# BarryFutureman/EvolutionaryDistributedTraining

Measured on AMD Instinct MI355X. Metric: GB/s of param bytes reduced per outer step (device-resident), 1/2/4/8 GPUs, higher is better.
Workload: dtype f32

## Files before the change

evolutionarydistributedtraining_amd/_lib.py:

```python
from __future__ import annotations

import ctypes
import os

import torch

PKG_DIR = os.path.dirname(os.path.abspath(__file__))
LIB_PATH = os.path.join(PKG_DIR, "libedt_sync.so")

EDT_F32 = 0
EDT_BF16 = 1
EDT_MAX_WORKERS = 64
EDT_MXFP8 = 0
EDT_MXFP4 = 1
EDT_ROUND_NEAREST = 0
EDT_ROUND_STOCHASTIC = 1
EDT_ABI_VERSION = 6

_DT = {torch.float32: EDT_F32, torch.bfloat16: EDT_BF16}

_P = ctypes.c_void_p
_U64 = ctypes.c_uint64
_I = ctypes.c_int
_D = ctypes.c_double
SIGNATURES = [
    ("edt_outer_step", _I, [_P, _I, ctypes.POINTER(_P), _I, _I, _P, _I, _U64, _D, _D, _I, _P]),
    ("edt_outer_step_bcast", _I, [_P, _I, ctypes.POINTER(_P), _I, _I, _P, _I, _U64, _D, _D, _I,
                                  ctypes.POINTER(_P), _I, _P]),
    ("edt_outer_step_tail", _I, [_P, _I, ctypes.POINTER(_P), _I, _I, _P, _I, _U64, _D, _D, _I, _P, _P]),
    ("edt_outer_step_scaled", _I, [_P, _I, ctypes.POINTER(_P), _I, _I, _P, _I, _U64, _D, _D, _I, _P,
                                   ctypes.c_float, _P]),
    ("edt_delta_stats_doubles", _U64, [_I, ctypes.c_int64]),
    ("edt_delta_stats", _I, [_P, _I, ctypes.POINTER(_P), _I, _I, _U64, _P, ctypes.c_int64, _P, _P]),
    ("edt_pair_merge_tail", _I, [_P, _P, _P, _P, _I, _P, _I, _P, _P, _I, _U64, _D, _D, _I, _P, _P]),
    ("edt_outer_step_ws", _I, [_P, _I, ctypes.POINTER(_P), _I, _I, _P, _I, _U64, _D, _D, _I, _P, _P]),
    ("edt_outer_list_workspace_bytes", _U64, [_I, _I]),
    ("edt_outer_step_list", _I, [ctypes.POINTER(_P), _I, ctypes.POINTER(_P), _I, _I, ctypes.POINTER(_P), _I,
                                 ctypes.POINTER(_U64), _I, _D, _D, _I, _P, _U64, _P]),
    ("edt_outer_step_list_tail", _I, [ctypes.POINTER(_P), _I, ctypes.POINTER(_P), _I, _I, ctypes.POINTER(_P), _I,
                                      ctypes.POINTER(_U64), _I, _D, _D, _I, _P, ctypes.POINTER(_U64), _P, _U64, _P]),
    ("edt_outer_step_list_scaled", _I, [ctypes.POINTER(_P), _I, ctypes.POINTER(_P), _I, _I, ctypes.POINTER(_P), _I,
                                        ctypes.POINTER(_U64), _I, _D, _D, _I, _P, ctypes.POINTER(_U64),
                                        ctypes.c_float, _P, _U64, _P]),
    ("edt_delta_stats_list_workspace_bytes", _U64, [_I, _I]),
    ("edt_delta_stats_list", _I, [ctypes.POINTER(_P), _I, ctypes.POINTER(_P), _I, _I, ctypes.POINTER(_U64), _I, _P,
                                  ctypes.c_int64, _P, _P, _U64, _P]),
    ("edt_delta_partial", _I, [_P, _I, ctypes.POINTER(_P), _I, _I, _I, _U64, _P, _I, _P]),
    ("edt_sgd_apply", _I, [_P, _I, _P, _P, _I, _U64, _D, _D, _I, _P]),
    ("edt_sgd_apply_sum", _I, [_P, _I, ctypes.POINTER(_P), _I, _P, _I, _U64, _D, _D, _I, _P]),
    ("edt_sgd_apply_scaled", _I, [_P, _I, _P, _P, _I, _U64, _D, _D, _I, ctypes.c_float, _P]),
    ("edt_sgd_apply_sum_scaled", _I, [_P, _I, ctypes.POINTER(_P), _I, _P, _I, _U64, _D, _D, _I, ctypes.c_float, _P]),
    ("edt_partial_sum_stats_doubles", _U64, [ctypes.c_int64]),
    ("edt_partial_sum_stats", _I, [ctypes.POINTER(_P), _I, _I, _U64, _P, ctypes.c_int64, _P, _P]),
    ("edt_q_region_bytes", _U64, [_U64, _I]),
    ("edt_delta_partial_q", _I, [_P, _I, ctypes.POINTER(_P), _I, _I, _I, _U64, _U64, _I, _P, _P, _P]),
    ("edt_sgd_apply_sum_q", _I, [_P, _I, ctypes.POINTER(_P), _I, _I, _P, _I, _U64, _D, _D, _I, _P]),
# ... 171 lines not shown
```

evolutionarydistributedtraining_amd/csrc/edt_outer.hip:

```cpp
#include "edt_step.h"

namespace {


struct Workers {
    const void* p[EDT_MAX_WORKERS];
};

struct OuterArgs {
    void* theta;
    void* mom;
    float* acc_out;
    uint64_t n;
    int K;
    float kdiv;
    float kinv;
    int div_exact;
    int accumulate;
    void* acc_ws;
    int acc_in;
    int acc_store;
    SgdScalars sgd;
    Workers w;
    Workers bc;
// ... 183 lines not shown
};

template <int GDT, int N, bool SC = false, class... S>
__global__ __launch_bounds__(kBlock) void sgd_apply_sum_kernel(void* theta, Partials P, int np, void* mom,
                                                               uint64_t n, SgdScalars s, S... scale) {
    static_assert(sizeof...(S) == (SC ? 1 : 0), "one grad_scale with SC, none without");
    for_vec_tail<N>(n, [&](auto tagN, uint64_t i) {
        constexpr int M = decltype(tagN)::value;
        float g0[M], g[M];
        sgd_from_sum<GDT, M, SC>(theta, mom, i, s, np, [&](int r, float (&x)[M]) { ld<EDT_F32, M>(P.p[r], i, x); }, g0, g,
                                 scale...);
        st<GDT, M>(theta, i, g);
    });
}

template <int GDT, int N, bool SC = false, class... S>
__global__ __launch_bounds__(kBlock) void sgd_apply_kernel(void* theta, const float* acc, void* mom,
                                                           uint64_t n, SgdScalars s, S... scale) {
    static_assert(sizeof...(S) == (SC ? 1 : 0), "one grad_scale with SC, none without");
    for_vec_tail<N>(n, [&](auto tagN, uint64_t i) {
        constexpr int M = decltype(tagN)::value;
        float g0[M], g[M];
        sgd_from_sum<GDT, M, SC>(theta, mom, i, s, 1, [&](int, float (&x)[M]) { ld<EDT_F32, M>(acc, i, x); }, g0, g,
                                 scale...);
        st<GDT, M>(theta, i, g);
    });
}



template <int GDT, int WDT, int KC, int N, int H2 = 4>
__device__ __forceinline__ void probe_elems(const OuterArgs& a, uint64_t i) {
    float g[N], b[N], acc[N];
    ld<GDT, N, false, H2>(a.theta, i, g);
    ld<GDT, N, false, H2>(a.mom, i, b);
#pragma unroll
    for (int j = 0; j < N; ++j) acc[j] = 0.f;
    const int K = KC > 0 ? KC : a.K;
#pragma unroll 8
    for (int k = 0; k < K; ++k) {
        float w[N];
        ld<WDT, N, nt_worker_loads<WDT, H2>(), H2>(a.wp(k), i, w);
#pragma unroll
        for (int j = 0; j < N; ++j) acc[j] += w[j];
    }
#pragma unroll
// ... 455 lines not shown
    return sgd_apply_sum_impl<false>(theta_g, gdt, acc_f32, nacc, momentum, has_momentum, n, lr, momentum_coef, nesterov,
                                     1.f, stream);
}

int edt_sgd_apply_sum_scaled(void* theta_g, int gdt, const float* const* acc_f32, int nacc, void* momentum,
                             int has_momentum, uint64_t n, double lr, double momentum_coef, int nesterov,
                             float grad_scale, void* stream) {
    return sgd_apply_sum_impl<true>(theta_g, gdt, acc_f32, nacc, momentum, has_momentum, n, lr, momentum_coef, nesterov,
                                    grad_scale, stream);
}

int edt_sgd_apply(void* theta_g, int gdt, const float* acc_f32, void* momentum, int has_momentum,
                  uint64_t n, double lr, double momentum_coef, int nesterov, void* stream) {
    return sgd_apply_impl<false>(theta_g, gdt, acc_f32, momentum, has_momentum, n, lr, momentum_coef, nesterov, 1.f,
                                 stream);
}

int edt_sgd_apply_scaled(void* theta_g, int gdt, const float* acc_f32, void* momentum, int has_momentum,
                         uint64_t n, double lr, double momentum_coef, int nesterov, float grad_scale, void* stream) {
    return sgd_apply_impl<true>(theta_g, gdt, acc_f32, momentum, has_momentum, n, lr, momentum_coef, nesterov,
                                grad_scale, stream);
}

}
```

evolutionarydistributedtraining_amd/csrc/edt_stats.hip:

```cpp
#include "edt_chunksum.h"
#include "edt_mx.h"
#include "edt_step.h"

namespace {

constexpr int kStatsGroup = 8;
constexpr int kStatsUpc = kTileSlots / kWavesPerBlock;
constexpr int kStatsMaxWidth = 3 * EDT_MAX_WORKERS + 2;

__host__ __device__ constexpr int stats_width(int K) { return 3 * K + 2; }

struct StatsWorkers {
    const void* p[EDT_MAX_WORKERS];
};

struct StatsArgs {
    const void* theta;
    const uint64_t* chunks;
    double* rows;
    uint64_t units;
    uint64_t u0;
    int K;
    float kdiv;
    float kinv;
    StatsWorkers w;
    static constexpr bool kList = false;
    __device__ __forceinline__ const StatsArgs& operands(uint64_t) const { return *this; }
    __device__ __forceinline__ const void* th() const { return theta; }
    __device__ __forceinline__ const void* wp(int k) const { return w.p[k]; }
};

struct StatsListArgs;
struct TensorOperands {
    const StatsListArgs& a;
    uint64_t t;
    __device__ __forceinline__ const void* th() const;
    __device__ __forceinline__ const void* wp(int k) const;
};

struct StatsListArgs {
    const void* const* theta;
    const void* const* w;
    const uint64_t* vec;
    const uint64_t* chunks;
    double* rows;
    uint64_t units;
    uint64_t u0;
    uint64_t T;
    int K;
    float kdiv;
    float kinv;
    static constexpr bool kList = true;
    __device__ __forceinline__ TensorOperands operands(uint64_t c) const { return {*this, chunks[3 * c + 2]}; }
};
__device__ __forceinline__ const void* TensorOperands::th() const { return a.theta[t]; }
__device__ __forceinline__ const void* TensorOperands::wp(int k) const { return a.w[(uint64_t)k * a.T + t]; }


template <int DT, bool VEC, bool NT>
__device__ __forceinline__ void ld8(const void* p, uint64_t i, float (&x)[kVec]) {
    if constexpr (VEC) {
        ld<DT, kVec, NT>(p, i, x);
    } else {
#pragma unroll
        for (int j = 0; j < kVec; ++j) {
            float y[1];
            ld<DT, 1>(p, i + j, y);
            x[j] = y[0];
        }
    }
}

template <int N>
__device__ __forceinline__ void mask_count(float (&x)[N], double& count) {
#pragma unroll
    for (int j = 0; j < N; ++j) {
        const bool bad = (__float_as_uint(x[j]) & 0x7fffffffu) >= 0x7f800000u;
        if (bad) {
            x[j] = 0.f;
            count += 1.0;
        }
    }
}

template <int N>
__device__ __forceinline__ void dot_chain(const float (&x)[N], const float (&y)[N], double& s) {
#pragma unroll
    for (int j = 0; j < N; ++j) s = __builtin_fma((double)x[j], (double)y[j], s);
}

template <int GDT, int WDT, int DIV, int KC, bool KM, bool VEC, class Args>
__global__ __launch_bounds__(kBlock) void delta_stats_kernel(Args a) {
// ... 34 lines not shown
        for (int q = 0; q < G; ++q) {
#pragma unroll
            for (int j = 0; j < kVec; ++j) d[q][j] = 0.f;
            de[q][0] = 0.f;
            if (KC > 0 ? q < KC : k0 + q < K) {
                if (has_vec) ld8<WDT, VEC, NT>(o.wp(k0 + q), i, d[q]);
                if (has_edge) ld<WDT, 1>(o.wp(k0 + q), e, de[q]);
            }
        }
#pragma unroll
        for (int q = 0; q < G; ++q) {
            if (KC > 0 ? q < KC : k0 + q < K) {
                delta_of<GDT>(d[q], g);
                mean_add<GDT, DIV, true>(a, d[q], acc);
                delta_of<GDT>(de[q], ge);
                mean_add<GDT, DIV, true>(a, de[q], acce);
                mask_count(d[q], ck[q]);
                mask_count(de[q], ck[q]);
                dot_chain(d[q], d[q], skk[q]);
                dot_chain(de[q], de[q], skk[q]);
            }
        }
        if constexpr (KM) {
            mask_count(acc, cm);
            mask_count(acce, cm);
            dot_chain(acc, acc, smm);
            dot_chain(acce, acce, smm);
#pragma unroll
            for (int q = 0; q < G; ++q) {
                dot_chain(d[q], acc, skm[q]);
                dot_chain(de[q], acce, skm[q]);
            }
            double v[3 * G + 2], r[Red<3 * G + 2>::N2];
            v[0] = smm;
            v[2 * G + 1] = cm;
#pragma unroll
            for (int q = 0; q < G; ++q) {
                v[1 + q] = skk[q];
                v[1 + G + q] = skm[q];
                v[2 * G + 2 + q] = ck[q];
            }
            tile_reduce<3 * G + 2>(v, r);
            red_store<3 * G + 2>(r, [&](int idx, double x) {
                if (idx == 0) row[0] = x;
                else if (idx <= G) { if (idx - 1 < K) row[idx] = x; }
                else if (idx <= 2 * G) { if (idx - 1 - G < K) row[K + idx - G] = x; }
                else if (idx == 2 * G + 1) row[2 * K + 1] = x;
                else if (idx - 2 * G - 2 < K) row[2 * K + idx - 2 * G] = x;
            });
        } else {
            double v[2 * G], r[Red<2 * G>::N2];
#pragma unroll
            for (int q = 0; q < G; ++q) {
                v[q] = skk[q];
                v[G + q] = ck[q];
            }
            tile_reduce<2 * G>(v, r);
            red_store<2 * G>(r, [&](int idx, double x) {
                const int k = k0 + (idx < G ? idx : idx - G);
                if (k < K) row[(idx < G ? 1 : 2 * K + 2) + k] = x;
            });
        }
    }
    if constexpr (!KM) {
        mask_count(acc, cm);
        mask_count(acce, cm);
        dot_chain(acc, acc, smm);
        dot_chain(acce, acce, smm);
        const double v[2] = {smm, cm};
        double r[Red<2>::N2];
        tile_reduce<2>(v, r);
        red_store<2>(r, [&](int idx, double x) { row[idx == 0 ? 0 : 2 * K + 1] = x; });
    }
    __syncthreads();
    const int W = stats_width(K);
    double* out = a.rows + unit_slot(u, a.units) * (uint64_t)W;
    for (int q = threadIdx.x; q < W; q += kBlock) {
        double x = 0.0;
        if (KM || q <= K || q > 2 * K) x = (part[0][q] + part[1][q]) + (part[2][q] + part[3][q]);
        out[q] = x;
    }
}

template <int GDT, int WDT, int DIV, int KC, bool KM, bool VEC, class A>
int launch_stats(A a, hipStream_t s) {
    const uint64_t units = a.units;
    for (uint64_t u0 = 0; u0 < units; u0 += kUnitGridCap) {
// ... 142 lines not shown
    const double v[2] = {smm, cm};
    double r[Red<2>::N2];
    tile_reduce<2>(v, r);
    red_store<2>(r, [&](int idx, double x) { part[wave][idx] = x; });
    __syncthreads();
    double* out = a.rows + unit_slot(u, a.units) * (uint64_t)kPartialStatsWidth;
    if (threadIdx.x < kPartialStatsWidth) {
        const int q = threadIdx.x;
        out[q] = (part[0][q] + part[1][q]) + (part[2][q] + part[3][q]);
    }
}

template <int GDT, int FMT, int NPC>
int launch_partial_stats_q(PartialStatsQArgs a, hipStream_t s) {
    const uint64_t units = a.units;
    for (uint64_t u0 = 0; u0 < units; u0 += kUnitGridCap) {
        a.u0 = u0;
        partial_sum_stats_q_kernel<GDT, FMT, NPC><<<unit_grid(units - u0), kBlock, 0, s>>>(a);
        if (int rc = check_launch("partial_sum_stats_q_kernel")) return rc;
    }
    return EDT_OK;
}

}

extern "C" {

uint64_t edt_partial_sum_stats_doubles(int64_t nchunks) {
    if (nchunks < 0) return 0;
    return (uint64_t)nchunks * (uint64_t)kPartialStatsWidth * (1ull + kStatsUpc);
}

int edt_partial_sum_stats(const float* const* acc_f32, int nacc, int gdt, uint64_t n, const uint64_t* chunk_desc,
                          int64_t nchunks, double* out, void* stream) {
    g_err[0] = 0;
    int rc = check_master_dtype(gdt);
    if (!rc) rc = check_partial_count(nacc);
    if (rc) return rc;
    if (nchunks < 0) return fail(EDT_ERR_ARG, "negative chunk count");
    if (!acc_f32) return fail(EDT_ERR_ARG, "acc_f32 is null");
    if (n == 0 || nchunks == 0) return EDT_OK;
    if (!chunk_desc || !out) return fail(EDT_ERR_ARG, "null chunk table or output");
    if (reinterpret_cast<uintptr_t>(out) & 7u) return fail(EDT_ERR_ARG, "out must be 8-byte aligned");
    PartialStatsArgs a;
    memset(&a, 0, sizeof(a));
    bool vec = true;
// ... 49 lines not shown
        constexpr int GD = decltype(G)::value;
        return with_fmt(fmt, [&](auto F) {
            constexpr int FM = decltype(F)::value;
            switch (nacc) {
                case 1: return launch_partial_stats_q<GD, FM, 1>(a, s);
                case 2: return launch_partial_stats_q<GD, FM, 2>(a, s);
                case 4: return launch_partial_stats_q<GD, FM, 4>(a, s);
                case 8: return launch_partial_stats_q<GD, FM, 8>(a, s);
                default: return launch_partial_stats_q<GD, FM, 0>(a, s);
            }
        });
    });
    if (rc) return rc;
    return launch_tree_reduce(a.rows, kPartialStatsWidth, kStatsUpc, kStatsUpc, 1, nchunks, out, s);
}

uint64_t edt_delta_stats_doubles(int K, int64_t nchunks) {
    if (K < 1 || K > EDT_MAX_WORKERS || nchunks < 0) return 0;
    return (uint64_t)nchunks * (uint64_t)stats_width(K) * (1ull + kStatsUpc);
}

int edt_delta_stats(const void* theta_g, int gdt, const void* const* theta_k, int wdt, int K, uint64_t n,
                    const uint64_t* chunk_desc, int64_t nchunks, double* out, void* stream) {
    g_err[0] = 0;
    if (!valid_pair(gdt, wdt)) return fail(EDT_ERR_ARG, "unsupported dtype pair (gdt/wdt)");
    if (K < 1 || K > EDT_MAX_WORKERS)
        return fail(EDT_ERR_ARG, "worker count %d out of range [1, %d]", K, EDT_MAX_WORKERS);
    if (nchunks < 0) return fail(EDT_ERR_ARG, "negative chunk count");
    if (!theta_k) return fail(EDT_ERR_ARG, "theta_k is null");
    if (n == 0 || nchunks == 0) return EDT_OK;
    if (!theta_g) return fail(EDT_ERR_ARG, "theta_g is null");
    if (!chunk_desc || !out) return fail(EDT_ERR_ARG, "null chunk table or output");
    if (reinterpret_cast<uintptr_t>(out) & 7u) return fail(EDT_ERR_ARG, "out must be 8-byte aligned");
    StatsArgs a;
    memset(&a, 0, sizeof(a));
    bool vec = aligned16(theta_g);
    for (int k = 0; k < K; ++k) {
        if (!theta_k[k]) return fail(EDT_ERR_ARG, "theta_k[%d] is null", k);
        a.w.p[k] = theta_k[k];
        vec = vec && aligned16(theta_k[k]);
    }
    a.theta = theta_g;
    a.chunks = chunk_desc;
    a.rows = out + (uint64_t)nchunks * stats_width(K);
    a.units = (uint64_t)nchunks * kStatsUpc;
    a.K = K;
    a.kdiv = (float)K;
    a.kinv = 1.0f / (float)K;
    return dispatch_stats(a, Bool<false>{}, gdt, wdt, vec, nchunks, out, (hipStream_t)stream);
}

uint64_t edt_delta_stats_list_workspace_bytes(int T, int K) {
    if (T < 0 || K < 1 || K > EDT_MAX_WORKERS) return 0;
    return ((uint64_t)K + 2) * (uint64_t)T * sizeof(uint64_t);
}

int edt_delta_stats_list(const void* const* theta_t, int gdt, const void* const* theta_k, int wdt, int K,
                         const uint64_t* numel, int T, const uint64_t* chunk_desc, int64_t nchunks, double* out,
                         void* workspace, uint64_t workspace_bytes, void* stream) {
    g_err[0] = 0;
    if (!valid_pair(gdt, wdt)) return fail(EDT_ERR_ARG, "unsupported dtype pair (gdt/wdt)");
    if (K < 1 || K > EDT_MAX_WORKERS)
        return fail(EDT_ERR_ARG, "worker count %d out of range [1, %d]", K, EDT_MAX_WORKERS);
    if (T < 0) return fail(EDT_ERR_ARG, "tensor count %d < 0", T);
    if (nchunks < 0) return fail(EDT_ERR_ARG, "negative chunk count");
    if (T == 0 || nchunks == 0) return EDT_OK;
    if (!theta_t || !theta_k || !numel) return fail(EDT_ERR_ARG, "null tensor table");
    if (!chunk_desc || !out) return fail(EDT_ERR_ARG, "null chunk table or output");
    if (reinterpret_cast<uintptr_t>(out) & 7u) return fail(EDT_ERR_ARG, "out must be 8-byte aligned");
    const uint64_t need = edt_delta_stats_list_workspace_bytes(T, K);
    if (!workspace || workspace_bytes < need)
        return fail(EDT_ERR_ARG, "workspace of %llu bytes needed", (unsigned long long)need);
// ... 44 lines not shown
```

evolutionarydistributedtraining_amd/diloco.py:

```python
from __future__ import annotations

import os

import torch

from . import ops
from ._lib import EDT_MAX_WORKERS as L_MAX, EdtError
from .guard import NonFiniteWorkers, OuterGuard, clip_coefficient, guard_decision, stats_totals
from .guard import fold_remeasured, report
from .params import ParamArena, ParamLayout, flat_view, pack, unpack_
from .tracing import traced

DILOCO_DEFAULTS = dict(lr=0.7, momentum=0.9, nesterov=True)


def check_sgd_hparams(lr: float, momentum: float, nesterov: bool) -> None:
    if lr < 0.0:
        raise ValueError(f"Invalid learning rate: {lr}")
    if momentum < 0.0:
        raise ValueError(f"Invalid momentum value: {momentum}")
    if nesterov and momentum <= 0:
        raise ValueError("Nesterov momentum requires a momentum and zero dampening")
DILOCO_SIM_DEFAULTS = dict(lr=1.0, momentum=0.0, nesterov=False)


class OuterState:

    def __init__(self, place_momentum: int = 0):
        self.momentum: torch.Tensor | None = None
        self.has_momentum = False
        self.hparams = dict(DILOCO_DEFAULTS)
        self.steps = 0
        self.place_momentum = int(place_momentum)
        self.placement: dict | None = None
        self.last_stats: dict | None = None

    def buffer_for(self, theta: torch.Tensor, numel: int | None = None) -> torch.Tensor:
        numel = theta.numel() if numel is None else numel
        if self.momentum is None:
            self.momentum = torch.zeros(numel, dtype=theta.dtype, device=theta.device)
            self.has_momentum = False
        elif self.momentum.numel() != numel:
            raise EdtError("outer-optimizer state does not match the parameter count "
                           f"({self.momentum.numel()} vs {numel})")
        elif self.momentum.dtype != theta.dtype or self.momentum.device != theta.device:
            self.momentum = self.momentum.to(dtype=theta.dtype, device=theta.device)
        return self.momentum

    def state_dict(self, layout: ParamLayout) -> dict:
        state = {}
        if self.momentum is not None and self.has_momentum:
            for i, v in enumerate(layout.views(self.momentum)):
                state[i] = {"momentum_buffer": v.detach().to("cpu", copy=True)}
        group = dict(lr=self.hparams["lr"], momentum=self.hparams["momentum"], dampening=0,
                     weight_decay=0, nesterov=self.hparams["nesterov"], maximize=False,
                     foreach=None, differentiable=False, fused=None,
                     params=list(range(len(layout))))
        return {"state": state, "param_groups": [group]}
# ... 15 lines not shown
    def save(self, path: str, layout: ParamLayout) -> None:
        torch.save(self.state_dict(layout), path)

    @classmethod
    def load(cls, path: str, layout: ParamLayout, dtype, device) -> "OuterState":
        st = cls()
        st.load_state_dict(torch.load(path, map_location="cpu", weights_only=True), layout, dtype, device)
        return st


def _stats_plan(state, theta: torch.Tensor, numels):
    offs = [0]
    for n in (numels if numels is not None else [theta.numel()]):
        offs.append(offs[-1] + int(n))
    if offs[-1] != theta.numel():
        raise EdtError("the guard's per-tensor sizes do not add up to theta's size")
    key = (tuple(offs), str(theta.device))
    cached = getattr(state, "_stats_plan", None)
    if cached is None or cached[0] != key:
        cached = state._stats_plan = (key, ops.make_slerp_plan(offs, theta.device))
    return cached[1]


def _measure(theta, workers, plan, per_tensor: bool) -> dict:
    rows = ops.delta_stats(theta, workers, plan).cpu().numpy()
    first = plan.seg_first.cpu().numpy() if per_tensor else None
    return stats_totals(rows, len(workers), first)


def _stats_list_plan(state, thetas):
    offs = [0]
    for t in thetas:
        offs.append(offs[-1] + t.numel())
    key = (tuple(offs), str(thetas[0].device))
    cached = getattr(state, "_stats_list_plan", None)
    if cached is None or cached[0] != key:
        cached = state._stats_list_plan = (key, ops.make_slerp_plan(offs, thetas[0].device, relative=True))
    return cached[1]


def _measure_list(thetas, workers, plan, per_tensor: bool) -> dict:
    rows = ops.delta_stats_list(thetas, workers, plan).cpu().numpy()
    first = plan.seg_first.cpu().numpy() if per_tensor else None
    return stats_totals(rows, len(workers), first)


def _guard_pass(theta, workers, state, guard: OuterGuard, numels):
    if len(workers) > L_MAX:
        raise EdtError(f"a guarded step takes at most {L_MAX} workers")
    plan = _stats_plan(state, theta, numels if guard.per_tensor else None)
    return _guard_decide(lambda ws: _measure(theta, ws, plan, guard.per_tensor), workers, state, guard)


def _guard_pass_list(thetas, workers, state, guard: OuterGuard):
    if len(workers) > L_MAX:
        raise EdtError(f"a guarded step takes at most {L_MAX} workers")
    plan = _stats_list_plan(state, thetas)
    return _guard_decide(lambda ws: _measure_list(thetas, ws, plan, guard.per_tensor), workers, state, guard)


def _guard_decide(measure, workers, state, guard: OuterGuard):
    K = len(workers)
    first = measure(workers)
    rep = state.last_stats = dict(report(first), clip_coef=None, dropped=[])
    survivors, clip = guard_decision(first, guard)
    final = first
    if clip is None:
        final = measure([workers[k] for k in survivors])
        rep["dropped"] = [k for k in range(K) if k not in survivors]
        fold_remeasured(rep, report(final), survivors, K)
        _, clip = guard_decision(final, guard)
        if clip is None:
            raise EdtError("the survivors' statistics flagged a worker")
    if guard.per_tensor:
# ... 2 lines not shown
    return survivors, clip


def _tail_bits(cpu_tails, numels, device, state=None, per_tensor=False):
    if cpu_tails is None:
        return None
    key = (tuple(int(n) for n in numels), tuple(cpu_tails), str(device), per_tensor)
    cached = getattr(state, "_tail_cache", None) if state is not None else None
    if cached is not None and cached[0] == key:
        return cached[1]
    from .torchcompat import torch_cpu_tail_bits, torch_cpu_tail_bits_per_tensor
    vec, threads = cpu_tails
    if per_tensor:
        got = torch_cpu_tail_bits_per_tensor(numels, vec_elems=vec, num_threads=threads, device=device)
    else:
        got = torch_cpu_tail_bits(numels, vec_elems=vec, num_threads=threads, device=device)
    if state is not None:
        state._tail_cache = (key, got)
    return got


def _step_flat(theta: torch.Tensor, workers: list[torch.Tensor], state: OuterState, lr: float,
               momentum: float, nesterov: bool, broadcast: list[torch.Tensor] | None = None,
               tail_bits: torch.Tensor | None = None, guard: OuterGuard | None = None, numels=None) -> None:
    check_sgd_hparams(lr, momentum, nesterov)
    clip = 1.0
    if guard is not None:
        survivors, clip = _guard_pass(theta, workers, state, guard, numels)
        workers = [workers[k] for k in survivors]
    state.hparams = dict(lr=lr, momentum=momentum, nesterov=nesterov)
    fresh = state.momentum is None
    mom = state.buffer_for(theta) if momentum != 0 else None
    if mom is not None and fresh and getattr(state, "place_momentum", 0) > 1 and theta.is_cuda:
        from .placement import place_momentum
        try:
            state.momentum, state.placement = place_momentum(theta, workers, mom, state.place_momentum)
            mom = state.momentum
        except EdtError as e:
            state.placement = {"candidates": 1, "probe_ms": [], "chosen": 0, "skipped": str(e)}
    has = state.has_momentum if momentum != 0 else False
    if clip != 1.0:
        ops.outer_step_scaled(theta, workers, mom, has, lr, momentum, nesterov, clip, tail_bits=tail_bits)
        if broadcast:
            ops.broadcast_theta(theta, broadcast)
    elif tail_bits is not None and broadcast:
        ops.outer_step(theta, workers, mom, has, lr, momentum, nesterov, tail_bits=tail_bits)
        for b in broadcast:
            b.copy_(theta)
    else:
        ops.outer_step(theta, workers, mom, has, lr, momentum, nesterov, broadcast, tail_bits=tail_bits)
    if momentum != 0:
        state.has_momentum = True
    state.steps += 1


def _step_list(thetas: list[torch.Tensor], workers: list[list[torch.Tensor]], state: OuterState,
               lr: float, momentum: float, nesterov: bool, tails=None, guard: OuterGuard | None = None) -> None:
    check_sgd_hparams(lr, momentum, nesterov)
    clip = 1.0
    if guard is not None:
        survivors, clip = _guard_pass_list(thetas, workers, state, guard)
        workers = [workers[k] for k in survivors]
    state.hparams = dict(lr=lr, momentum=momentum, nesterov=nesterov)
    moms = None
# ... 32 lines not shown
        theta = flat_view(base_params)
        flats = [flat_view(w) for w in worker_params]
        if guard is not None and len(worker_params) > L_MAX:
            raise EdtError(f"a guarded step takes at most {L_MAX} workers")
        if theta is None or any(f is None for f in flats):
            bf16_master = base_params and base_params[0].dtype == torch.bfloat16
            if (cpu_tails is None or bf16_master) and len(worker_params) <= L_MAX and base_params \
                    and all(p.is_cuda for p in base_params):
                if len({w[0].dtype for w in worker_params}) != 1:
                    raise EdtError("all trained models must share one dtype")
                tails = _tail_bits(cpu_tails, [p.numel() for p in base_params], base_params[0].device, state,
                                   per_tensor=True)
                _step_list(base_params, worker_params, state, lr, momentum, nesterov, tails=tails, guard=guard)
                return state
        copied = theta is None
        if copied:
            theta = pack(base_params)
        flats = [f if f is not None else pack(w) for f, w in zip(flats, worker_params)]
        wdt = {f.dtype for f in flats}
        if len(wdt) != 1:
            raise EdtError("all trained models must share one dtype")
        _step_flat(theta, flats, state, lr, momentum, nesterov,
                   tail_bits=_tail_bits(cpu_tails, [p.numel() for p in base_params], theta.device, state),
                   guard=guard, numels=[p.numel() for p in base_params])
        if copied:
            unpack_(theta, base_params)
    return state


class OuterSync:

    def __init__(self, theta: ParamArena, workers: list[ParamArena], lr: float = 0.7,
                 momentum: float = 0.9, nesterov: bool = True, state: OuterState | None = None,
                 cpu_tails: tuple[int, int] | None = None, guard: OuterGuard | None = None):
        if guard is not None and len(workers) > L_MAX:
            raise EdtError(f"a guarded step takes at most {L_MAX} workers")
        self.guard = guard
        self.theta = theta
        self.workers = workers
        self.lr, self.momentum, self.nesterov = lr, momentum, nesterov
        self.state = state or OuterState()
        self.tail_bits = _tail_bits(cpu_tails, theta.layout.numels, theta.flat.device)

    @traced("edt/OuterSync.step")
    def step(self, broadcast: bool = False) -> None:
        ws = [w.flat for w in self.workers]
        _step_flat(self.theta.flat, ws, self.state, self.lr, self.momentum, self.nesterov,
                   ws if broadcast else None, tail_bits=self.tail_bits, guard=self.guard,
                   numels=self.theta.layout.numels)

    @property
    def last_stats(self) -> dict | None:
        return self.state.last_stats

    def place_momentum(self, candidates: int = 8) -> dict:
        if self.momentum == 0:
            return {"candidates": 0, "probe_ms": [], "chosen": None}
        from .placement import place_momentum
        mom = self.state.buffer_for(self.theta.flat)
        self.state.momentum, rep = place_momentum(self.theta.flat, [w.flat for w in self.workers], mom,
                                                  candidates)
        return rep

    def place_arenas(self, draws: int = 3, candidates: int = 8) -> dict:
        if self.momentum == 0:
            return {"draws": [], "chosen_draw": None}
        from .placement import place_set
        mom = self.state.buffer_for(self.theta.flat)
        th, ws, m, rep = place_set(self.theta.flat, [w.flat for w in self.workers], mom, draws, candidates)
        self.theta.flat = th
        for w, f in zip(self.workers, ws):
            w.flat = f
        self.state.momentum = m
        return rep

    def broadcast_(self) -> None:
        for w in self.workers:
            w.flat.copy_(self.theta.flat)

    @property
    def bytes_reduced(self) -> int:
        return sum(w.flat.numel() * w.flat.element_size() for w in self.workers)

    def traffic_bytes(self) -> int:
        n = self.theta.flat.numel()
        b = self.bytes_reduced + 2 * n * self.theta.flat.element_size()
        if self.momentum != 0:
            b += (2 if self.state.has_momentum else 1) * n * self.theta.flat.element_size()
        return b


class DirOuterSync:

    INNER_STATE_FILES = ("optimizer.pt", "scheduler.pt")

    def __init__(self, device=None, theta_dtype=None, worker_dtype=None, names=None,
# ... 95 lines not shown
```

evolutionarydistributedtraining_amd/ops.py:

```python
from __future__ import annotations

import ctypes
import threading
from dataclasses import dataclass

import numpy as np
import torch

from . import _lib as L


def outer_step(theta: torch.Tensor, workers: list[torch.Tensor], momentum: torch.Tensor | None,
               has_momentum: bool, lr: float, momentum_coef: float, nesterov: bool,
               broadcast: list[torch.Tensor] | None = None, tail_bits: torch.Tensor | None = None) -> None:
    lib = L.lib()
    n = theta.numel()
    head = _step_head(theta, workers, momentum, has_momentum, lr, momentum_coef, nesterov, *(broadcast or []))
    if broadcast and any(b.numel() != n or b.dtype != workers[0].dtype for b in broadcast):
        raise L.EdtError("broadcast buffers must match theta's size and the workers' dtype")
    if tail_bits is not None:
        _check_tail_bits(tail_bits, n)
        if len(workers) > L.EDT_MAX_WORKERS:
            raise L.EdtError("tail emulation runs in the plain fused step (<= 64 workers)")
        L.check(lib.edt_outer_step_tail(*head, L.ptr(tail_bits), L.stream_ptr(theta.device)), "edt_outer_step_tail")
# ... 13 lines not shown
        L.check(lib.edt_outer_step(*head, L.stream_ptr(theta.device)), "edt_outer_step")
        return
    ws = torch.empty_like(theta)
    L.check(lib.edt_outer_step_ws(*head, L.ptr(ws), L.stream_ptr(theta.device)), "edt_outer_step_ws")


def outer_step_scaled(theta: torch.Tensor, workers: list[torch.Tensor], momentum: torch.Tensor | None,
                      has_momentum: bool, lr: float, momentum_coef: float, nesterov: bool, grad_scale: float,
                      tail_bits: torch.Tensor | None = None) -> None:
    lib = L.lib()
    head = _step_head(theta, workers, momentum, has_momentum, lr, momentum_coef, nesterov)
    if len(workers) > L.EDT_MAX_WORKERS:
        raise L.EdtError(f"the scaled step takes at most {L.EDT_MAX_WORKERS} workers")
    _check_tail_bits(tail_bits, theta.numel())
    L.check(lib.edt_outer_step_scaled(*head, L.ptr(tail_bits), float(grad_scale), L.stream_ptr(theta.device)),
            "edt_outer_step_scaled")


def stats_columns(K: int) -> dict:
    return {"S_mm": slice(0, 1), "S_kk": slice(1, K + 1), "S_km": slice(K + 1, 2 * K + 1),
            "nonfinite_mean": slice(2 * K + 1, 2 * K + 2), "nonfinite": slice(2 * K + 2, 3 * K + 2)}


def delta_stats(theta: torch.Tensor, workers: list[torch.Tensor], plan: "SlerpPlan") -> torch.Tensor:
    lib = L.lib()
    if not workers:
        raise L.EdtError("no workers")
    L.require_device(theta, *workers)
    n, K = theta.numel(), len(workers)
    _check_workers(theta, workers)
    if K > L.EDT_MAX_WORKERS:
        raise L.EdtError(f"the statistics pass takes at most {L.EDT_MAX_WORKERS} workers")
    _check_stats_plan(plan, n, theta.device, "theta's")
    W = 3 * K + 2
    out = _scratch(theta.device, int(lib.edt_delta_stats_doubles(K, plan.nchunks)))
    L.check(lib.edt_delta_stats(L.ptr(theta), L.dtype_code(theta), L.ptr_array(workers), L.dtype_code(workers[0]),
                                K, n, L.ptr(plan.chunks), plan.nchunks, L.ptr(out), L.stream_ptr(theta.device)),
            "edt_delta_stats")
    return out[:plan.nchunks * W].view(plan.nchunks, W)


def delta_stats_list(thetas: list[torch.Tensor], workers: list[list[torch.Tensor]], plan: "SlerpPlan") -> torch.Tensor:
    lib = L.lib()
    T, K = len(thetas), len(workers)
    if K == 0:
        raise L.EdtError("no workers")
    if K > L.EDT_MAX_WORKERS:
        raise L.EdtError(f"the statistics pass takes at most {L.EDT_MAX_WORKERS} workers")
    flat_w, numels, gdt, wdt = _check_list_operands(thetas, workers, None)
    if not plan.relative or plan.nseg != T or plan.seg_numel.tolist() != numels:
        raise L.EdtError("the chunk plan must be relative with one segment per tensor, of the tensors' sizes")
    W = 3 * K + 2
    if T == 0 or plan.nchunks == 0:
        return torch.zeros(0, W, dtype=torch.float64, device=thetas[0].device if T else plan.chunks.device)
    dev = thetas[0].device
    if plan.chunks.device != dev:
        raise L.EdtError("the chunk plan lives on another device")
    out = _scratch(dev, int(lib.edt_delta_stats_doubles(K, plan.nchunks)))
    nbytes = lib.edt_delta_stats_list_workspace_bytes(T, K)
    ws = torch.empty(nbytes, dtype=torch.uint8, device=dev)
    P_ = ctypes.c_void_p
# ... 1252 lines not shown
```

include/edt_sync.h:

```cpp
#ifndef EDT_SYNC_H
#define EDT_SYNC_H

#include <stdint.h>

#define EDT_ABI_VERSION 6

#ifdef __cplusplus
extern "C" {
#endif

int edt_abi_version(void);

typedef enum { EDT_F32 = 0, EDT_BF16 = 1 } edt_dtype_t;

enum {
    EDT_OK = 0,
    EDT_ERR_ARG = -1,
    EDT_ERR_LAUNCH = -2,
};

#define EDT_MAX_WORKERS 64

int edt_outer_step(void* theta_g, int gdt, const void* const* theta_k, int wdt, int K,
                   void* momentum, int has_momentum, uint64_t n,
                   double lr, double momentum_coef, int nesterov, void* stream);

int edt_outer_step_bcast(void* theta_g, int gdt, const void* const* theta_k, int wdt, int K,
                         void* momentum, int has_momentum, uint64_t n, double lr, double momentum_coef,
                         int nesterov, void* const* bcast, int nbcast, void* stream);

int edt_outer_step_tail(void* theta_g, int gdt, const void* const* theta_k, int wdt, int K,
                        void* momentum, int has_momentum, uint64_t n, double lr, double momentum_coef,
                        int nesterov, const uint8_t* tail_bits, void* stream);
int edt_pair_merge_tail(const void* b1, const void* b2, const void* m1, const void* m2, int wdt,
                        void* theta_out, int gdt, const void* momentum_in, void* momentum_out,
                        int has_momentum, uint64_t n, double lr, double momentum_coef, int nesterov,
                        const uint8_t* tail_bits, void* stream);

uint64_t edt_delta_stats_doubles(int K, int64_t nchunks);
int edt_delta_stats(const void* theta_g, int gdt, const void* const* theta_k, int wdt, int K, uint64_t n,
                    const uint64_t* chunk_desc, int64_t nchunks, double* out, void* stream);

int edt_outer_step_scaled(void* theta_g, int gdt, const void* const* theta_k, int wdt, int K,
                          void* momentum, int has_momentum, uint64_t n, double lr, double momentum_coef,
                          int nesterov, const uint8_t* tail_bits, float grad_scale, void* stream);

int edt_outer_step_ws(void* theta_g, int gdt, const void* const* theta_k, int wdt, int K,
                      void* momentum, int has_momentum, uint64_t n, double lr, double momentum_coef,
                      int nesterov, void* workspace, void* stream);

uint64_t edt_outer_list_workspace_bytes(int T, int K);
int edt_outer_step_list(void* const* theta_t, int gdt, const void* const* theta_k, int wdt, int K,
                        void* const* momentum_t, int has_momentum, const uint64_t* numel, int T,
                        double lr, double momentum, int nesterov, void* workspace,
                        uint64_t workspace_bytes, void* stream);
int edt_outer_step_list_tail(void* const* theta_t, int gdt, const void* const* theta_k, int wdt, int K,
                             void* const* momentum_t, int has_momentum, const uint64_t* numel, int T,
                             double lr, double momentum, int nesterov, const uint8_t* tail_bits,
                             const uint64_t* tail_byte_offset, void* workspace, uint64_t workspace_bytes,
                             void* stream);
int edt_outer_step_list_scaled(void* const* theta_t, int gdt, const void* const* theta_k, int wdt, int K,
                               void* const* momentum_t, int has_momentum, const uint64_t* numel, int T,
                               double lr, double momentum, int nesterov, const uint8_t* tail_bits,
                               const uint64_t* tail_byte_offset, float grad_scale, void* workspace,
                               uint64_t workspace_bytes, void* stream);

uint64_t edt_delta_stats_list_workspace_bytes(int T, int K);
int edt_delta_stats_list(const void* const* theta_t, int gdt, const void* const* theta_k, int wdt, int K,
// ... 209 lines not shown
```

Before: 4047.

## Carry worker mean from guard stats pass into outer step to skip re-reading workers

When a guard is active, the delta-stats kernel now also writes the per-element worker mean into a persistent workspace. If every worker survives and nothing is non-finite, the outer step applies SGD from that stored mean instead of re-reading all K worker buffers. This cuts the second K-way read over worker parameters, at the cost of an extra n-element write and read plus a persistent buffer the size of theta. It applies only to guarded OuterSync steps, where carry_mean now defaults to true.

```diff
diff --git a/evolutionarydistributedtraining_amd/_lib.py b/evolutionarydistributedtraining_amd/_lib.py
--- a/evolutionarydistributedtraining_amd/_lib.py
+++ b/evolutionarydistributedtraining_amd/_lib.py
@@ -32,6 +32,8 @@
                                    ctypes.c_float, _P]),
     ("edt_delta_stats_doubles", _U64, [_I, ctypes.c_int64]),
     ("edt_delta_stats", _I, [_P, _I, ctypes.POINTER(_P), _I, _I, _U64, _P, ctypes.c_int64, _P, _P]),
+    ("edt_delta_stats_mean", _I, [_P, _I, ctypes.POINTER(_P), _I, _I, _U64, _P, ctypes.c_int64, _P, _P, _P]),
+    ("edt_outer_apply_mean_scaled", _I, [_P, _I, _P, _P, _I, _U64, _D, _D, _I, _P, ctypes.c_float, _P]),
     ("edt_pair_merge_tail", _I, [_P, _P, _P, _P, _I, _P, _I, _P, _P, _I, _U64, _D, _D, _I, _P, _P]),
     ("edt_outer_step_ws", _I, [_P, _I, ctypes.POINTER(_P), _I, _I, _P, _I, _U64, _D, _D, _I, _P, _P]),
     ("edt_outer_list_workspace_bytes", _U64, [_I, _I]),
diff --git a/evolutionarydistributedtraining_amd/csrc/edt_outer.hip b/evolutionarydistributedtraining_amd/csrc/edt_outer.hip
--- a/evolutionarydistributedtraining_amd/csrc/edt_outer.hip
+++ b/evolutionarydistributedtraining_amd/csrc/edt_outer.hip
@@ -229,6 +229,19 @@
         constexpr int M = decltype(tagN)::value;
         float g0[M], g[M];
         sgd_from_sum<GDT, M, SC>(theta, mom, i, s, 1, [&](int, float (&x)[M]) { ld<EDT_F32, M>(acc, i, x); }, g0, g,
+                                 scale...);
+        st<GDT, M>(theta, i, g);
+    });
+}
+
+template <int GDT, int N, bool SC = false, class... S>
+__global__ __launch_bounds__(kBlock) void apply_mean_kernel(void* theta, const void* mean, void* mom, uint64_t n,
+                                                            SgdScalars s, S... scale) {
+    static_assert(sizeof...(S) == (SC ? 1 : 0), "one grad_scale with SC, none without");
+    for_vec_tail<N>(n, [&](auto tagN, uint64_t i) {
+        constexpr int M = decltype(tagN)::value;
+        float g0[M], g[M];
+        sgd_from_sum<GDT, M, SC>(theta, mom, i, s, 1, [&](int, float (&x)[M]) { ld<GDT, M>(mean, i, x); }, g0, g,
                                  scale...);
         st<GDT, M>(theta, i, g);
     });
@@ -730,4 +743,35 @@
                                 grad_scale, stream);
 }
 
-}
+int edt_outer_apply_mean_scaled(void* theta_g, int gdt, const void* mean, void* momentum, int has_momentum,
+                                uint64_t n, double lr, double momentum_coef, int nesterov, const uint8_t* tail_bits,
+                                float grad_scale, void* stream) {
+    g_err[0] = 0;
+    int rc = check_master_dtype(gdt);
+    if (!rc) rc = check_grad_scale(grad_scale);
+    if (rc) return rc;
+    if (n == 0) return EDT_OK;
+    if (!theta_g) return fail(EDT_ERR_ARG, "theta_g is null");
+    if (!mean) return fail(EDT_ERR_ARG, "mean is null");
+    SgdScalars s;
+    if ((rc = shard_sgd(s, gdt, lr, momentum_coef, has_momentum, nesterov, momentum))) return rc;
+    const uint64_t bytes = n * (gdt == EDT_BF16 ? 2 : 4);
+    if (bytes_overlap(mean, bytes, theta_g, bytes)) return fail(EDT_ERR_ARG, "mean overlaps theta_g");
+    if (s.use_momentum && bytes_overlap(mean, bytes, momentum, bytes)) return fail(EDT_ERR_ARG, "mean overlaps momentum");
+    if (gdt == EDT_BF16) s.tail = tail_bits;
+    const bool vec = aligned16(theta_g) && aligned16(mean) && (!s.use_momentum || aligned16(momentum));
+    const unsigned g = grid_for(n, vec);
+    hipStream_t st = (hipStream_t)stream;
+    return with_dtype(gdt, [&](auto G) {
+        return with_bool(vec, [&](auto V) {
+            constexpr int GD = decltype(G)::value, N = decltype(V)::value ? kVec : 1;
+            if (grad_scale != 1.f)
+                apply_mean_kernel<GD, N, true><<<g, kBlock, 0, st>>>(theta_g, mean, momentum, n, s, grad_scale);
+            else
+                apply_mean_kernel<GD, N><<<g, kBlock, 0, st>>>(theta_g, mean, momentum, n, s);
+            return check_launch("apply_mean_kernel");
+        });
+    });
+}
+
+}
diff --git a/evolutionarydistributedtraining_amd/csrc/edt_stats.hip b/evolutionarydistributedtraining_amd/csrc/edt_stats.hip
--- a/evolutionarydistributedtraining_amd/csrc/edt_stats.hip
+++ b/evolutionarydistributedtraining_amd/csrc/edt_stats.hip
@@ -25,9 +25,15 @@
     float kinv;
     StatsWorkers w;
     static constexpr bool kList = false;
+    static constexpr bool kMean = false;
     __device__ __forceinline__ const StatsArgs& operands(uint64_t) const { return *this; }
     __device__ __forceinline__ const void* th() const { return theta; }
     __device__ __forceinline__ const void* wp(int k) const { return w.p[k]; }
+};
+
+struct StatsArgsMean : StatsArgs {
+    void* mean;
+    static constexpr bool kMean = true;
 };
 
 struct StatsListArgs;
@@ -51,6 +57,7 @@
     float kdiv;
     float kinv;
     static constexpr bool kList = true;
+    static constexpr bool kMean = false;
     __device__ __forceinline__ TensorOperands operands(uint64_t c) const { return {*this, chunks[3 * c + 2]}; }
 };
 __device__ __forceinline__ const void* TensorOperands::th() const { return a.theta[t]; }
@@ -68,6 +75,25 @@
             ld<DT, 1>(p, i + j, y);
             x[j] = y[0];
         }
+    }
+}
+
+template <int GDT, bool VEC, class Args>
+__device__ __forceinline__ void store_mean(const Args& a, bool has_vec, uint64_t i, const float (&acc)[kVec],
+                                           bool has_edge, uint64_t e, const float (&acce)[1]) {
+    if constexpr (Args::kMean) {
+        if (has_vec) {
+            if constexpr (VEC) {
+                st<GDT, kVec>(a.mean, i, acc);
+            } else {
+#pragma unroll
+                for (int j = 0; j < kVec; ++j) {
+                    const float y[1] = {acc[j]};
+                    st<GDT, 1>(a.mean, i + j, y);
+                }
+            }
+        }
+        if (has_edge) st<GDT, 1>(a.mean, e, acce);
     }
 }
 
@@ -148,6 +174,7 @@
             }
         }
         if constexpr (KM) {
+            store_mean<GDT, VEC>(a, has_vec, i, acc, has_edge, e, acce);
             mask_count(acc, cm);
             mask_count(acce, cm);
             dot_chain(acc, acc, smm);
@@ -189,6 +216,7 @@
         }
     }
     if constexpr (!KM) {
+        store_mean<GDT, VEC>(a, has_vec, i, acc, has_edge, e, acce);
         mask_count(acc, cm);
         mask_count(acce, cm);
         dot_chain(acc, acc, smm);
@@ -377,6 +405,49 @@
     return EDT_OK;
 }
 
+}
+
+template <bool MEAN>
+static int delta_stats_impl(Bool<MEAN>, const void* theta_g, int gdt, const void* const* theta_k, int wdt, int K,
+                            uint64_t n, const uint64_t* chunk_desc, int64_t nchunks, double* out, void* mean_out,
+                            void* stream) {
+    g_err[0] = 0;
+    if (!valid_pair(gdt, wdt)) return fail(EDT_ERR_ARG, "unsupported dtype pair (gdt/wdt)");
+    if (K < 1 || K > EDT_MAX_WORKERS)
+        return fail(EDT_ERR_ARG, "worker count %d out of range [1, %d]", K, EDT_MAX_WORKERS);
+    if (nchunks < 0) return fail(EDT_ERR_ARG, "negative chunk count");
+    if (!theta_k) return fail(EDT_ERR_ARG, "theta_k is null");
+    if (n == 0 || nchunks == 0) return EDT_OK;
+    if (!theta_g) return fail(EDT_ERR_ARG, "theta_g is null");
+    if (!chunk_desc || !out) return fail(EDT_ERR_ARG, "null chunk table or output");
+    if (reinterpret_cast<uintptr_t>(out) & 7u) return fail(EDT_ERR_ARG, "out must be 8-byte aligned");
+    std::conditional_t<MEAN, StatsArgsMean, StatsArgs> a;
+    memset(&a, 0, sizeof(a));
+    bool vec = aligned16(theta_g);
+    for (int k = 0; k < K; ++k) {
+        if (!theta_k[k]) return fail(EDT_ERR_ARG, "theta_k[%d] is null", k);
+        a.w.p[k] = theta_k[k];
+        vec = vec && aligned16(theta_k[k]);
+    }
+    if constexpr (MEAN) {
+        if (!mean_out) return fail(EDT_ERR_ARG, "mean_out is null");
+        const uint64_t gb = n * (gdt == EDT_BF16 ? 2 : 4), wb = n * (wdt == EDT_BF16 ? 2 : 4);
+        if (bytes_overlap(mean_out, gb, theta_g, gb)) return fail(EDT_ERR_ARG, "mean_out overlaps theta_g");
+        for (int k = 0; k < K; ++k)
+            if (bytes_overlap(mean_out, gb, theta_k[k], wb)) return fail(EDT_ERR_ARG, "mean_out overlaps theta_k[%d]", k);
+        if (bytes_overlap(mean_out, gb, out, edt_delta_stats_doubles(K, nchunks) * sizeof(double)))
+            return fail(EDT_ERR_ARG, "mean_out overlaps out");
+        a.mean = mean_out;
+        vec = vec && aligned16(mean_out);
+    }
+    a.theta = theta_g;
+    a.chunks = chunk_desc;
+    a.rows = out + (uint64_t)nchunks * stats_width(K);
+    a.units = (uint64_t)nchunks * kStatsUpc;
+    a.K = K;
+    a.kdiv = (float)K;
+    a.kinv = 1.0f / (float)K;
+    return dispatch_stats(a, Bool<false>{}, gdt, wdt, vec, nchunks, out, (hipStream_t)stream);
 }
 
 extern "C" {
@@ -472,32 +543,12 @@
 
 int edt_delta_stats(const void* theta_g, int gdt, const void* const* theta_k, int wdt, int K, uint64_t n,
                     const uint64_t* chunk_desc, int64_t nchunks, double* out, void* stream) {
-    g_err[0] = 0;
-    if (!valid_pair(gdt, wdt)) return fail(EDT_ERR_ARG, "unsupported dtype pair (gdt/wdt)");
-    if (K < 1 || K > EDT_MAX_WORKERS)
-        return fail(EDT_ERR_ARG, "worker count %d out of range [1, %d]", K, EDT_MAX_WORKERS);
-    if (nchunks < 0) return fail(EDT_ERR_ARG, "negative chunk count");
-    if (!theta_k) return fail(EDT_ERR_ARG, "theta_k is null");
-    if (n == 0 || nchunks == 0) return EDT_OK;
-    if (!theta_g) return fail(EDT_ERR_ARG, "theta_g is null");
-    if (!chunk_desc || !out) return fail(EDT_ERR_ARG, "null chunk table or output");
-    if (reinterpret_cast<uintptr_t>(out) & 7u) return fail(EDT_ERR_ARG, "out must be 8-byte aligned");
-    StatsArgs a;
-    memset(&a, 0, sizeof(a));
-    bool vec = aligned16(theta_g);
-    for (int k = 0; k < K; ++k) {
-        if (!theta_k[k]) return fail(EDT_ERR_ARG, "theta_k[%d] is null", k);
-        a.w.p[k] = theta_k[k];
-        vec = vec && aligned16(theta_k[k]);
-    }
-    a.theta = theta_g;
-    a.chunks = chunk_desc;
-    a.rows = out + (uint64_t)nchunks * stats_width(K);
-    a.units = (uint64_t)nchunks * kStatsUpc;
-    a.K = K;
-    a.kdiv = (float)K;
-    a.kinv = 1.0f / (float)K;
-    return dispatch_stats(a, Bool<false>{}, gdt, wdt, vec, nchunks, out, (hipStream_t)stream);
+    return delta_stats_impl(Bool<false>{}, theta_g, gdt, theta_k, wdt, K, n, chunk_desc, nchunks, out, nullptr, stream);
+}
+
+int edt_delta_stats_mean(const void* theta_g, int gdt, const void* const* theta_k, int wdt, int K, uint64_t n,
+                         const uint64_t* chunk_desc, int64_t nchunks, double* out, void* mean_out, void* stream) {
+    return delta_stats_impl(Bool<true>{}, theta_g, gdt, theta_k, wdt, K, n, chunk_desc, nchunks, out, mean_out, stream);
 }
 
 uint64_t edt_delta_stats_list_workspace_bytes(int T, int K) {
diff --git a/evolutionarydistributedtraining_amd/diloco.py b/evolutionarydistributedtraining_amd/diloco.py
--- a/evolutionarydistributedtraining_amd/diloco.py
+++ b/evolutionarydistributedtraining_amd/diloco.py
@@ -34,6 +34,14 @@
         self.place_momentum = int(place_momentum)
         self.placement: dict | None = None
         self.last_stats: dict | None = None
+        self.mean_ws: torch.Tensor | None = None
+        self.mean_carried = False
+
+    def give_mean_workspace(self, theta: torch.Tensor) -> torch.Tensor:
+        ws = self.mean_ws
+        if ws is None or ws.numel() != theta.numel() or ws.dtype != theta.dtype or ws.device != theta.device:
+            ws = self.mean_ws = torch.empty(theta.numel(), dtype=theta.dtype, device=theta.device)
+        return ws
 
     def buffer_for(self, theta: torch.Tensor, numel: int | None = None) -> torch.Tensor:
         numel = theta.numel() if numel is None else numel
@@ -95,8 +103,8 @@
     return cached[1]
 
 
-def _measure(theta, workers, plan, per_tensor: bool) -> dict:
-    rows = ops.delta_stats(theta, workers, plan).cpu().numpy()
+def _measure(theta, workers, plan, per_tensor: bool, mean_out=None) -> dict:
+    rows = ops.delta_stats(theta, workers, plan, mean_out=mean_out).cpu().numpy()
     first = plan.seg_first.cpu().numpy() if per_tensor else None
     return stats_totals(rows, len(workers), first)
 
@@ -118,11 +126,23 @@
     return stats_totals(rows, len(workers), first)
 
 
-def _guard_pass(theta, workers, state, guard: OuterGuard, numels):
+def _guard_pass(theta, workers, state, guard: OuterGuard, numels, mean_ws=None):
     if len(workers) > L_MAX:
         raise EdtError(f"a guarded step takes at most {L_MAX} workers")
     plan = _stats_plan(state, theta, numels if guard.per_tensor else None)
-    return _guard_decide(lambda ws: _measure(theta, ws, plan, guard.per_tensor), workers, state, guard)
+    return _guard_decide(lambda ws: _measure(theta, ws, plan, guard.per_tensor, mean_ws if ws is workers else None),
+                         workers, state, guard)
+
+
+def _fitting(mean_ws, theta: torch.Tensor):
+    if mean_ws is None or mean_ws.numel() != theta.numel() or mean_ws.dtype != theta.dtype \
+            or mean_ws.device != theta.device:
+        return None
+    return mean_ws
+
+
+def _mean_usable(rep: dict, survivors, K: int) -> bool:
+    return len(survivors) == K and not rep["dropped"] and rep["nonfinite_mean"] == 0 and not any(rep["nonfinite"])
 
 
 def _guard_pass_list(thetas, workers, state, guard: OuterGuard):
@@ -171,11 +191,16 @@
 
 def _step_flat(theta: torch.Tensor, workers: list[torch.Tensor], state: OuterState, lr: float,
                momentum: float, nesterov: bool, broadcast: list[torch.Tensor] | None = None,
-               tail_bits: torch.Tensor | None = None, guard: OuterGuard | None = None, numels=None) -> None:
+               tail_bits: torch.Tensor | None = None, guard: OuterGuard | None = None, numels=None,
+               mean_ws: torch.Tensor | None = None) -> None:
     check_sgd_hparams(lr, momentum, nesterov)
     clip = 1.0
+    carried = False
     if guard is not None:
-        survivors, clip = _guard_pass(theta, workers, state, guard, numels)
+        K = len(workers)
+        survivors, clip = _guard_pass(theta, workers, state, guard, numels, mean_ws)
+        carried = mean_ws is not None and _mean_usable(state.last_stats, survivors, K)
+        state.mean_carried = carried
         workers = [workers[k] for k in survivors]
     state.hparams = dict(lr=lr, momentum=momentum, nesterov=nesterov)
     fresh = state.momentum is None
@@ -188,7 +213,11 @@
         except EdtError as e:
             state.placement = {"candidates": 1, "probe_ms": [], "chosen": 0, "skipped": str(e)}
     has = state.has_momentum if momentum != 0 else False
-    if clip != 1.0:
+    if carried:
+        ops.outer_apply_mean(theta, mean_ws, mom, has, lr, momentum, nesterov, clip, tail_bits=tail_bits)
+        if broadcast:
+            ops.broadcast_theta(theta, broadcast)
+    elif clip != 1.0:
         ops.outer_step_scaled(theta, workers, mom, has, lr, momentum, nesterov, clip, tail_bits=tail_bits)
         if broadcast:
             ops.broadcast_theta(theta, broadcast)
@@ -267,7 +296,7 @@
             raise EdtError("all trained models must share one dtype")
         _step_flat(theta, flats, state, lr, momentum, nesterov,
                    tail_bits=_tail_bits(cpu_tails, [p.numel() for p in base_params], theta.device, state),
-                   guard=guard, numels=[p.numel() for p in base_params])
+                   guard=guard, numels=[p.numel() for p in base_params], mean_ws=_fitting(state.mean_ws, theta))
         if copied:
             unpack_(theta, base_params)
     return state
@@ -277,22 +306,27 @@
 
     def __init__(self, theta: ParamArena, workers: list[ParamArena], lr: float = 0.7,
                  momentum: float = 0.9, nesterov: bool = True, state: OuterState | None = None,
-                 cpu_tails: tuple[int, int] | None = None, guard: OuterGuard | None = None):
+                 cpu_tails: tuple[int, int] | None = None, guard: OuterGuard | None = None,
+                 carry_mean: bool = True):
         if guard is not None and len(workers) > L_MAX:
             raise EdtError(f"a guarded step takes at most {L_MAX} workers")
         self.guard = guard
+        self.carry_mean = bool(carry_mean) and guard is not None
         self.theta = theta
         self.workers = workers
         self.lr, self.momentum, self.nesterov = lr, momentum, nesterov
         self.state = state or OuterState()
         self.tail_bits = _tail_bits(cpu_tails, theta.layout.numels, theta.flat.device)
+        if self.carry_mean:
+            self.state.give_mean_workspace(theta.flat)
 
     @traced("edt/OuterSync.step")
     def step(self, broadcast: bool = False) -> None:
         ws = [w.flat for w in self.workers]
         _step_flat(self.theta.flat, ws, self.state, self.lr, self.momentum, self.nesterov,
                    ws if broadcast else None, tail_bits=self.tail_bits, guard=self.guard,
-                   numels=self.theta.layout.numels)
+                   numels=self.theta.layout.numels,
+                   mean_ws=self.state.give_mean_workspace(self.theta.flat) if self.carry_mean else None)
 
     @property
     def last_stats(self) -> dict | None:
@@ -312,11 +346,14 @@
             return {"draws": [], "chosen_draw": None}
         from .placement import place_set
         mom = self.state.buffer_for(self.theta.flat)
+        self.state.mean_ws = None
         th, ws, m, rep = place_set(self.theta.flat, [w.flat for w in self.workers], mom, draws, candidates)
         self.theta.flat = th
         for w, f in zip(self.workers, ws):
             w.flat = f
         self.state.momentum = m
+        if self.carry_mean:
+            self.state.give_mean_workspace(th)
         return rep
 
     def broadcast_(self) -> None:
diff --git a/evolutionarydistributedtraining_amd/ops.py b/evolutionarydistributedtraining_amd/ops.py
--- a/evolutionarydistributedtraining_amd/ops.py
+++ b/evolutionarydistributedtraining_amd/ops.py
@@ -59,11 +59,27 @@
             "nonfinite_mean": slice(2 * K + 1, 2 * K + 2), "nonfinite": slice(2 * K + 2, 3 * K + 2)}
 
 
-def delta_stats(theta: torch.Tensor, workers: list[torch.Tensor], plan: "SlerpPlan") -> torch.Tensor:
+def outer_apply_mean(theta: torch.Tensor, mean: torch.Tensor, momentum: torch.Tensor | None, has_momentum: bool,
+                     lr: float, momentum_coef: float, nesterov: bool, grad_scale: float = 1.0,
+                     tail_bits: torch.Tensor | None = None) -> None:
+    lib = L.lib()
+    L.require_device(theta, mean, momentum)
+    if mean.dtype != theta.dtype or mean.numel() != theta.numel():
+        raise L.EdtError("mean must have theta's size and dtype")
+    _check_momentum(momentum, theta)
+    _check_tail_bits(tail_bits, theta.numel())
+    L.check(lib.edt_outer_apply_mean_scaled(L.ptr(theta), L.dtype_code(theta), L.ptr(mean), L.ptr(momentum),
+                                            int(has_momentum), theta.numel(), float(lr), float(momentum_coef),
+                                            int(nesterov), L.ptr(tail_bits), float(grad_scale),
+                                            L.stream_ptr(theta.device)), "edt_outer_apply_mean_scaled")
+
+
+def delta_stats(theta: torch.Tensor, workers: list[torch.Tensor], plan: "SlerpPlan",
+                mean_out: torch.Tensor | None = None) -> torch.Tensor:
     lib = L.lib()
     if not workers:
         raise L.EdtError("no workers")
-    L.require_device(theta, *workers)
+    L.require_device(theta, mean_out, *workers)
     n, K = theta.numel(), len(workers)
     _check_workers(theta, workers)
     if K > L.EDT_MAX_WORKERS:
@@ -71,9 +87,14 @@
     _check_stats_plan(plan, n, theta.device, "theta's")
     W = 3 * K + 2
     out = _scratch(theta.device, int(lib.edt_delta_stats_doubles(K, plan.nchunks)))
-    L.check(lib.edt_delta_stats(L.ptr(theta), L.dtype_code(theta), L.ptr_array(workers), L.dtype_code(workers[0]),
-                                K, n, L.ptr(plan.chunks), plan.nchunks, L.ptr(out), L.stream_ptr(theta.device)),
-            "edt_delta_stats")
+    head = (L.ptr(theta), L.dtype_code(theta), L.ptr_array(workers), L.dtype_code(workers[0]), K, n,
+            L.ptr(plan.chunks), plan.nchunks, L.ptr(out))
+    if mean_out is None:
+        L.check(lib.edt_delta_stats(*head, L.stream_ptr(theta.device)), "edt_delta_stats")
+    else:
+        if mean_out.dtype != theta.dtype or mean_out.numel() != n:
+            raise L.EdtError("mean_out must have theta's size and dtype")
+        L.check(lib.edt_delta_stats_mean(*head, L.ptr(mean_out), L.stream_ptr(theta.device)), "edt_delta_stats_mean")
     return out[:plan.nchunks * W].view(plan.nchunks, W)
 
 
diff --git a/include/edt_sync.h b/include/edt_sync.h
--- a/include/edt_sync.h
+++ b/include/edt_sync.h
@@ -44,6 +44,12 @@
 int edt_outer_step_scaled(void* theta_g, int gdt, const void* const* theta_k, int wdt, int K,
                           void* momentum, int has_momentum, uint64_t n, double lr, double momentum_coef,
                           int nesterov, const uint8_t* tail_bits, float grad_scale, void* stream);
+
+int edt_delta_stats_mean(const void* theta_g, int gdt, const void* const* theta_k, int wdt, int K, uint64_t n,
+                         const uint64_t* chunk_desc, int64_t nchunks, double* out, void* mean_out, void* stream);
+int edt_outer_apply_mean_scaled(void* theta_g, int gdt, const void* mean, void* momentum, int has_momentum,
+                                uint64_t n, double lr, double momentum_coef, int nesterov, const uint8_t* tail_bits,
+                                float grad_scale, void* stream);
 
 int edt_outer_step_ws(void* theta_g, int gdt, const void* const* theta_k, int wdt, int K,
                       void* momentum, int has_momentum, uint64_t n, double lr, double momentum_coef,
```

After: 3989. 0.986x the previous value.
